# loicland/superpoint_graph

Measured on AMD Instinct MI355X. Metric: superpoints/sec (embed+ECC fwd+bwd), S3DIS-shaped SPG, higher is better.
Workload: dtype f32; 1 GPU; gru_10_0,f_13 fwd+bwd+Adam; 1 scene/GPU x 1000 sp x 128 pts x 14 f, 5000 edges x 13 f; hipgraph=False, step_call=spg_train_step (one library call: forward + backward), parallelism=single GPU, batchnorm=per-rank statistics, precision=f32

## Files before the change

### superpoint_graph_amd/csrc/spg_gemm.hip

```cpp
#pragma clang fp contract(off)
#include "../../include/spg_hip.h"
#include "spg_gemm.h"
#include <type_traits>
#include <float.h>
#include <limits.h>
#include <stdarg.h>

static thread_local char g_err[512] = "";
extern "C" const char* spg_last_error(void) { return g_err; }
void spg_set_error(const char* fmt, ...) {
  va_list ap;
  va_start(ap, fmt);
  vsnprintf(g_err, sizeof(g_err), fmt, ap);
  va_end(ap);
}

#include <mutex>
#include <vector>
#ifdef SPG_ATTRIBUTION
#define SPG_DBG(p) ((p).dbg)
#else
#define SPG_DBG(p) 0
#endif
namespace {
// ... 122 lines not shown
};
static_assert(sizeof(SpgMultiArgs) <= 4096, "kernel arguments of a grouped launch must fit 4 KiB");
static_assert(sizeof(SpgGemmParams) % 8 == 0 && sizeof(SpgWgradParams) % 8 == 0, "parameter structs are packed back to back");
constexpr int spg_gemm_variant(bool wred, int amode, bool full) {
  const int m = amode == -1 ? (full ? -1 : 4)
              : amode == SPG_PRO_IDENT ? (full ? 1 : 0)
              : ((!wred && amode == SPG_PRO_AFFINE) || (wred && amode == SPG_PRO_BNBWD)) ? (full ? 3 : 2) : -1;
  return m < 0 ? -1 : (wred ? 5 : 0) + m;
}
constexpr bool spg_gemm_variant_light(int v) { return v != 8; }
#define SPG_WGRAD_VARIANTS(X)                                                                                    \
  X(0, 128, 128, 2, 2, 3, 1, false, false, false)   X(1, 128, 128, 2, 2, 3, 1, true, false, false)               \
  X(2, 64, 64, 2, 2, 0, 1, false, true, true)       X(3, 64, 64, 2, 2, 0, 1, true, true, true)                   \
  X(4, 128, 64, 2, 2, 0, 1, false, false, false)    X(5, 128, 64, 2, 2, 0, 1, true, false, false)                \
  X(6, 128, 128, 2, 2, -1, -1, false, true, false)                                                               \
  X(7, 128, 32, 4, 1, 0, 0, false, false, true)     X(8, 128, 32, 4, 1, 0, 0, true, false, true)                 \
  X(9, 128, 32, 4, 1, -1, -1, false, true, false)                                                                \
  X(10, 128, 32, 4, 1, 0, 0, false, true, false)    X(11, 128, 32, 4, 1, 0, 0, true, true, true)                 \
  X(12, 128, 32, 4, 1, 0, 1, false, true, false)    X(13, 128, 32, 4, 1, 0, 1, true, true, false)                \
  X(14, 64, 64, 2, 2, 0, 1, false, false, true)     X(15, 64, 64, 2, 2, 0, 1, true, false, true)                 \
  X(16, 128, 128, 2, 2, 0, 1, false, true, false)   X(17, 128, 128, 2, 2, 0, 1, true, true, false)               \
  X(18, 128, 64, 2, 2, 3, 1, false, false, false)   X(19, 128, 64, 2, 2, 3, 1, true, false, false)
constexpr int spg_wgrad_variant(int it, int jt, int amode, int bmode, bool full, bool colsum) {
#define SPG_X(id, IT_, JT_, WI_, WJ_, AM_, BM_, FU_, CS_, LI_) \
  if (it == IT_ && jt == JT_ && amode == AM_ && bmode == BM_ && full == FU_ && colsum == CS_) return id;
  SPG_WGRAD_VARIANTS(SPG_X)
#undef SPG_X
  return -1;
}
constexpr bool spg_wgrad_variant_light(int v) {
#define SPG_X(id, IT_, JT_, WI_, WJ_, AM_, BM_, FU_, CS_, LI_) if (v == id) return LI_;
  SPG_WGRAD_VARIANTS(SPG_X)
#undef SPG_X
  return false;
}
static bool spg_group_accepts(hipStream_t stream);
static bool spg_group_add(int kind, int variant, const void* params, size_t bytes, dim3 grid, size_t lds, double flops, hipStream_t stream, int weight,
                          std::function<int()> direct = nullptr);

__device__ __forceinline__ int spg_opaque_zero() { int z = 0; asm volatile("" : "+v"(z)); return z; }
template <typename T> using spg_kernarg_ptr = __attribute__((address_space(4))) const T*;
template <int BYTES>
__device__ __forceinline__ void spg_touch_params(const spg_kernarg_ptr<unsigned> b) {
  unsigned acc = 0;
#pragma unroll
  for (int o = 0; o < BYTES; o += 64) acc |= b[o / 4];
  asm volatile("" :: "s"(acc));
}
#define SPG_EPI_PIECE_ROWS 16
#define SPG_EPI_WAVE_FLOATS(RW, CW) (SPG_EPI_PIECE_ROWS * ((CW) + 8))

template <int RW, int CW, int TI, int TJ>
__device__ __forceinline__ void spg_store_tile_vec_impl(const f32x16 (&acc)[TI][TJ], float* __restrict__ st,
                                                        float* __restrict__ ybase, unsigned ldy, int lane) {
  constexpr int LD = CW + 8, LPR = CW / 4, RPI = 64 / LPR;
  static_assert(SPG_EPI_PIECE_ROWS % RPI == 0, "a piece is a whole number of store instructions");
  const int r = lane & 31, h = lane >> 5;
  const int lr = lane / LPR, lc = 4 * (lane % LPR);
  const unsigned o0 = (unsigned)lr * ldy + (unsigned)lc;
#pragma unroll
  for (int i = 0; i < TI; ++i)
#pragma unroll
    for (int half = 0; half < 2; ++half) {
#pragma unroll
      for (int j = 0; j < TJ; ++j)
#pragma unroll
        for (int u = 0; u < 8; ++u) st[((u & 3) + 8 * (u >> 2) + 4 * h) * LD + 32 * j + r] = acc[i][j][8 * half + u];
#pragma unroll
      for (int it = 0; it < SPG_EPI_PIECE_ROWS / RPI; ++it) {
        const f32x4 v = *reinterpret_cast<const f32x4*>(st + (lr + RPI * it) * LD + lc);
        __builtin_nontemporal_store(v, reinterpret_cast<f32x4*>(ybase + o0 + (unsigned)(32 * i + 16 * half + RPI * it) * ldy));
      }
    }
}
template <int RW, int CW, int TI, int TJ>
__device__ __forceinline__ void spg_store_tile_vec(const f32x16 (&acc)[TI][TJ], float* __restrict__ st,
                                                   float* __restrict__ ybase, unsigned ldy, int lane) {
  static_assert(TI * 32 == RW && TJ * 32 == CW, "wave sub-tile");
  spg_store_tile_vec_impl<RW, CW, TI, TJ>(acc, st, ybase, ldy, lane);
}

#include "spg_fold.h"

template <int TJ>
struct SpgStatAcc {
  float n;
  float a[TJ], b[TJ];
  f32x4 s1, s2;
  float sg[TJ];
  bool has_sg;
};

template <int IT, int JT, int WI, int WJ, bool FULL, bool BIAS_DONE = false>
__device__ __forceinline__ void spg_epilogue_fwd(const SpgGemmParams& p, f32x16 (&acc)[IT / WI / 32][JT / WJ / 32],
                                                 float* __restrict__ red, int tile, long m0, int mvalid, int n0,
                                                 SpgStatAcc<JT / WJ / 32>& sacc, const bool accum, unsigned long long* edbg = nullptr) {
  constexpr int TI = IT / WI / 32, TJ = JT / WJ / 32;
  const int tid = threadIdx.x + spg_opaque_zero(), lane = tid & 63, wave = tid >> 6;
  const int r = lane & 31, h = lane >> 5;
  const int wi = wave / WJ, wj = wave % WJ;
  const int colw = wj * (JT / WJ), roww = wi * (IT / WI);
#ifdef SPG_ATTRIBUTION
  unsigned long long et__ = __builtin_readcyclecounter();
#define SPG_EP(k) if (edbg != nullptr) { const unsigned long long n__ = __builtin_readcyclecounter(); edbg[k] += n__ - et__; et__ = n__; }
#else
#define SPG_EP(k)
#endif
#pragma unroll
  for (int j = 0; j < TJ; ++j) {
    const int col = n0 + colw + 32 * j + r;
    const bool colok = FULL || col < p.N;
    if (!BIAS_DONE && p.bias != nullptr) {
      const float t = p.bias[colok ? col : 0];
      const float bv = colok ? t : 0.f;
#pragma unroll
      for (int i = 0; i < TI; ++i)
#pragma unroll
        for (int q = 0; q < 16; ++q) acc[i][j][q] += bv;
    }
    if (p.Y != nullptr && !(FULL && p.vec_store)) {
      float* yb = p.Y + m0 * p.ldy + n0;
      const unsigned ldy = (unsigned)p.ldy;
      const unsigned o0 = (unsigned)(roww + 4 * h) * ldy + (unsigned)(colw + 32 * j + r);
#pragma unroll
      for (int i = 0; i < TI; ++i)
#pragma unroll
        for (int q = 0; q < 16; ++q) {
          const int row = 32 * i + spg_acc_row(q, h);
          if (FULL || (colok && roww + row < mvalid)) yb[o0 + (unsigned)(32 * i + (q & 3) + 8 * (q >> 2)) * ldy] = acc[i][j][q];
        }
    }
  }
  if (FULL && p.vec_store && p.Y != nullptr) {
    spg_store_tile_vec<IT / WI, JT / WJ>(acc, red + wave * SPG_EPI_WAVE_FLOATS(IT / WI, JT / WJ),
                                         p.Y + (m0 + roww) * p.ldy + n0 + colw, (unsigned)p.ldy, lane);
  }
  SPG_EP(0);
  const int nvw = min(max(mvalid - roww, 0), IT / WI);
  const long part = (long)tile * WI + wi;
  if (p.stat != nullptr || p.stat_slots != nullptr) {
    const float inv = nvw > 0 ? 1.f / (float)nvw : 0.f;
#pragma unroll
    for (int j = 0; j < TJ; ++j) {
      const int col = n0 + colw + 32 * j + r;
      float s = 0.f;
#pragma unroll
      for (int i = 0; i < TI; ++i)
#pragma unroll
        for (int q = 0; q < 16; ++q)
          if (FULL || roww + 32 * i + spg_acc_row(q, h) < mvalid) s += acc[i][j][q];
      s += __shfl_xor(s, 32, 64);
      const float mean = s * inv;
      float m2 = 0.f;
      if constexpr (FULL) {
        const spg_f32x2 mean2 = {mean, mean};
#pragma unroll
        for (int i = 0; i < TI; ++i)
#pragma unroll
          for (int q = 0; q < 16; q += 2) {
            const spg_f32x2 d = spg_f32x2{acc[i][j][q], acc[i][j][q + 1]} - mean2;
            m2 = fmaf(d[0], d[0], m2);
            m2 = fmaf(d[1], d[1], m2);
          }
      } else {
#pragma unroll
        for (int i = 0; i < TI; ++i)
#pragma unroll
          for (int q = 0; q < 16; ++q)
            if (roww + 32 * i + spg_acc_row(q, h) < mvalid) {
              const float d = acc[i][j][q] - mean;
              m2 = fmaf(d, d, m2);
            }
      }
      m2 += __shfl_xor(m2, 32, 64);
      if (accum) {
        const float na = sacc.n, nb = (float)nvw, nn = na + nb;
        const float delta = mean - sacc.a[j], f = nn > 0.f ? nb / nn : 0.f;
        sacc.a[j] += delta * f;
        sacc.b[j] += m2 + delta * delta * (na * f);
      } else if (h == 0 && (FULL || col < p.N)) {
        if (p.stat_slots != nullptr) {
          if (nvw > 0) spg_slots_add_fwd(p.stat_slots, p.N, col, (float)nvw, mean, m2);
        } else {
          p.stat[(part * 2 + 0) * p.N + col] = mean;
          p.stat[(part * 2 + 1) * p.N + col] = m2;
        }
      }
    }
    if (accum) sacc.n += (float)nvw;
    else if (lane == 0 && wj == 0 && n0 == 0 && p.stat_slots == nullptr) p.stat_cnt[part] = (float)nvw;
  }
  SPG_EP(1);
  if (p.pool_out != nullptr) {
    float* xch = red + 4 * SPG_EPI_WAVE_FLOATS(IT / WI, JT / WJ);
    int* xci = reinterpret_cast<int*>(xch + WI * JT);
    float* xsg = xch + 2 * WI * JT;
#pragma unroll
    for (int j = 0; j < TJ; ++j) {
      const int cl = colw + 32 * j + r, col = n0 + cl;
      const bool colok = FULL || col < p.N;
      const float sg = sacc.has_sg ? (sacc.sg[j] < 0.f ? -1.f : 1.f) : ((p.pool_sign != nullptr && p.pool_sign[colok ? col : 0] < 0.f) ? -1.f : 1.f);
      float kb = -FLT_MAX;
      int ib = INT_MAX;
      const spg_f32x2 sg2 = {sg, sg};
#pragma unroll
      for (int i = 0; i < TI; ++i)
#pragma unroll
        for (int q2 = 0; q2 < 16; q2 += 2) {
          const spg_f32x2 key2 = spg_f32x2{acc[i][j][q2], acc[i][j][q2 + 1]} * sg2;
#pragma unroll
          for (int e = 0; e < 2; ++e) {
            const int q = q2 + e;
            const int row = roww + 32 * i + spg_acc_row(q, h);
            const float key = key2[e];
            const bool gt = (FULL || row < mvalid) && key > kb;
            kb = gt ? key : kb; ib = gt ? row : ib;
          }
        }
      const float ok = __shfl_xor(kb, 32, 64);
      const int oi = __shfl_xor(ib, 32, 64);
      if (ok > kb || (ok == kb && oi < ib)) { kb = ok; ib = oi; }
      if (h == 0) { xch[wi * JT + cl] = kb; xci[wi * JT + cl] = ib; if (wi == 0) xsg[cl] = sg; }
    }
    SPG_EP(2);
    __syncthreads();
    for (int cl = tid; cl < JT; cl += SPG_THREADS) {
      const int col = n0 + cl;
      if (!FULL && col >= p.N) continue;
      float kb = xch[cl];
      int ib = xci[cl];
#pragma unroll
      for (int w = 1; w < WI; ++w) {
        const float ok = xch[w * JT + cl];
        const int oi = xci[w * JT + cl];
        if (ok > kb || (ok == kb && oi < ib)) { kb = ok; ib = oi; }
      }
      const float sg = xsg[cl];
      p.pool_out[(long)tile * p.pool_ld + col] = kb * sg;
      if (p.pool_idx != nullptr) p.pool_idx[(long)tile * p.pool_ld + col] = ib;
    }
    if (n0 == 0 && p.pool_extra != nullptr)
      for (int e = tid; e < p.pool_nextra; e += SPG_THREADS)
        p.pool_out[(long)tile * p.pool_ld + p.N + e] = p.pool_extra[(long)tile * p.pool_nextra + e];
    SPG_EP(3);
  }
}

template <int IT, int JT, int WI, int WJ>
__device__ __forceinline__ void spg_bwd_stat_store(const SpgGemmParams& p, f32x4 s1, f32x4 s2, long part, int n0) {
  constexpr int CW = JT / WJ, LPR = CW / 4;
  const int tid = threadIdx.x + spg_opaque_zero(), lane = tid & 63, wave = tid >> 6;
  const int wj = wave % WJ;
  const int col = n0 + wj * CW + 4 * (lane % LPR);
#pragma unroll
  for (int off = LPR; off < 64; off <<= 1) {
#pragma unroll
    for (int e = 0; e < 4; ++e) { s1[e] += __shfl_xor(s1[e], off, 64); s2[e] += __shfl_xor(s2[e], off, 64); }
  }
  if (lane < LPR) {
    if (p.stat_slots != nullptr) {
#pragma unroll
      for (int e = 0; e < 4; ++e)
        if (col + e < p.n_mask) spg_slots_add(p.stat_slots, p.n_mask, col + e, (double)s1[e], (double)s2[e]);
    } else {
      *reinterpret_cast<f32x4*>(p.stat + (part * 2 + 0) * p.N + col) = s1;
      *reinterpret_cast<f32x4*>(p.stat + (part * 2 + 1) * p.N + col) = s2;
    }
  }
}

template <int IT, int JT, int WI, int WJ>
__device__ __forceinline__ void spg_epilogue_bwd_vec(const SpgGemmParams& p, f32x16 (&acc)[IT / WI / 32][JT / WJ / 32],
                                                     float* __restrict__ red, int tile, long m0, int n0,
                                                     SpgStatAcc<JT / WJ / 32>& sacc, const bool accum) {
  constexpr int TI = IT / WI / 32, TJ = JT / WJ / 32, RW = IT / WI, CW = JT / WJ;
  constexpr int LD = CW + 8, LPR = CW / 4, RPI = 64 / LPR, NIT = SPG_EPI_PIECE_ROWS / RPI;
  static_assert(SPG_EPI_PIECE_ROWS % RPI == 0, "a piece is a whole number of store instructions");
  const int tid = threadIdx.x + spg_opaque_zero(), lane = tid & 63, wave = tid >> 6;
  const int r = lane & 31, h = lane >> 5;
  const int wi = wave / WJ, wj = wave % WJ;
  const int colw = wj * CW, roww = wi * RW;
  float* st = red + wave * SPG_EPI_WAVE_FLOATS(RW, CW);
  const bool do_stats = (p.stat != nullptr || p.stat_slots != nullptr) && p.mmean != nullptr;
  const bool do_mask = p.mask_relu != 0 && p.Yp != nullptr;
  const bool use_y = p.Yp != nullptr && (do_stats || do_mask);
  const int lr = lane / LPR, lc = 4 * (lane % LPR);
  const int col = n0 + colw + lc;
  f32x4 sc = {1.f, 1.f, 1.f, 1.f}, sh = {0.f, 0.f, 0.f, 0.f}, mean = sh, rstd = sh;
  if (p.ms != nullptr) { sc = *reinterpret_cast<const f32x4*>(p.ms + col); sh = *reinterpret_cast<const f32x4*>(p.mt + col); }
  if (do_stats) { mean = *reinterpret_cast<const f32x4*>(p.mmean + col); rstd = *reinterpret_cast<const f32x4*>(p.mrstd + col); }
  const float* yp = p.Yp + (m0 + roww) * p.ldyp + n0 + colw;
  float* yo = p.Y + (m0 + roww) * p.ldy + n0 + colw;
  const unsigned op0 = (unsigned)lr * (unsigned)p.ldyp + (unsigned)lc, oo0 = (unsigned)lr * (unsigned)p.ldy + (unsigned)lc;
  f32x4 s1 = {0.f, 0.f, 0.f, 0.f}, s2 = s1;
#pragma unroll
  for (int i = 0; i < TI; ++i)
#pragma unroll
    for (int half = 0; half < 2; ++half) {
      const int rb = 32 * i + 16 * half;
      f32x4 yv[NIT];
      if (use_y) {
#pragma unroll
        for (int u = 0; u < NIT; ++u) yv[u] = *reinterpret_cast<const f32x4*>(yp + op0 + (unsigned)(rb + RPI * u) * (unsigned)p.ldyp);
      }
#pragma unroll
      for (int j = 0; j < TJ; ++j)
#pragma unroll
        for (int u = 0; u < 8; ++u) st[((u & 3) + 8 * (u >> 2) + 4 * h) * LD + 32 * j + r] = acc[i][j][8 * half + u];
#pragma unroll
      for (int u = 0; u < NIT; ++u) {
        f32x4 v = *reinterpret_cast<const f32x4*>(st + (lr + RPI * u) * LD + lc);
        const f32x4 y = use_y ? yv[u] : f32x4{0.f, 0.f, 0.f, 0.f};
        if (do_mask) {
          const f32x4 act = spg_fma4(y, sc, sh);
#pragma unroll
          for (int e = 0; e < 4; ++e)
            if (!(act[e] > 0.f)) v[e] = 0.f;
        }
        if (do_stats) {
          s1 += v;
          s2 = spg_fma4(v, (y - mean) * rstd, s2);
        }
// ... 3 lines not shown
    }
  if (accum) {
    sacc.s1 += s1; sacc.s2 += s2;
  } else if (p.stat != nullptr || p.stat_slots != nullptr) {
    spg_bwd_stat_store<IT, JT, WI, WJ>(p, s1, s2, (long)tile * WI + wi, n0);
  }
}

template <int IT, int JT, int WI, int WJ, bool FULL>
__device__ __forceinline__ void spg_epilogue_bwd(const SpgGemmParams& p, f32x16 (&acc)[IT / WI / 32][JT / WJ / 32],
                                                 float* __restrict__ red, int tile, long m0, int mvalid, int n0) {
  constexpr int TI = IT / WI / 32, TJ = JT / WJ / 32;
  const int tid = threadIdx.x + spg_opaque_zero(), lane = tid & 63, wave = tid >> 6;
  const int r = lane & 31, h = lane >> 5;
  const int wi = wave / WJ, wj = wave % WJ;
  const int colw = wj * (JT / WJ), roww = wi * (IT / WI);
  const bool do_stats = (p.stat != nullptr || p.stat_slots != nullptr) && p.mmean != nullptr;
  const bool do_mask = p.mask_relu != 0 && p.Yp != nullptr;
  const bool use_y = p.Yp != nullptr && (do_stats || do_mask);
#pragma unroll
  for (int j = 0; j < TJ; ++j) {
    const int col = n0 + colw + 32 * j + r;
    const bool colok = FULL || col < p.N;
    const bool inm = FULL || col < p.n_mask;
    const int cc = (colok && inm) ? col : 0;
    float sc = 1.f, sh = 0.f, mean = 0.f, rstd = 0.f;
    if (p.ms != nullptr) { sc = p.ms[cc]; sh = p.mt[cc]; }
    if (do_stats) { mean = p.mmean[cc]; rstd = p.mrstd[cc]; }
    const float* yp = p.Yp + m0 * p.ldyp + n0;
    float* yo = p.Y + m0 * p.ldy + n0;
    const unsigned ldyp = (unsigned)p.ldyp, ldyo = (unsigned)p.ldy;
    const unsigned cl = (unsigned)(colw + 32 * j + r);
    const unsigned op0 = (unsigned)(roww + 4 * h) * ldyp + (colok ? cl : 0u);
    const unsigned oo0 = (unsigned)(roww + 4 * h) * ldyo + cl;
    float s1 = 0.f, s2 = 0.f;
#pragma unroll
    for (int i = 0; i < TI; ++i) {
      float yv[16];
      if (use_y) {
#pragma unroll
        for (int q = 0; q < 16; ++q) {
          const int row = 32 * i + spg_acc_row(q, h);
          const bool ok = FULL || (colok && roww + row < mvalid);
          yv[q] = yp[ok ? op0 + (unsigned)(32 * i + (q & 3) + 8 * (q >> 2)) * ldyp : 0u];
        }
      }
#pragma unroll
      for (int q = 0; q < 16; ++q) {
        const int row = 32 * i + spg_acc_row(q, h);
        const bool ok = FULL || (colok && roww + row < mvalid);
        float v = acc[i][j][q];
        const float y = use_y ? yv[q] : 0.f;
        if (do_mask && inm && !(fmaf(y, sc, sh) > 0.f)) v = 0.f;
        if (FULL || ok) yo[oo0 + (unsigned)(32 * i + (q & 3) + 8 * (q >> 2)) * ldyo] = v;
        if (do_stats) {
          const float w = (ok && inm) ? v : 0.f;
          s1 += w;
          s2 = fmaf(w, (y - mean) * rstd, s2);
        }
      }
      __builtin_amdgcn_sched_barrier(0);
    }
    if (p.stat != nullptr || p.stat_slots != nullptr) {
      s1 += __shfl_xor(s1, 32, 64);
      s2 += __shfl_xor(s2, 32, 64);
      if (h == 0 && (FULL || col < p.N)) {
        const long part = (long)tile * WI + wi;
        if (p.stat_slots != nullptr) {
          if (col < p.n_mask) spg_slots_add(p.stat_slots, p.n_mask, col, (double)s1, (double)s2);
        } else {
          p.stat[(part * 2 + 0) * p.N + col] = s1;
          p.stat[(part * 2 + 1) * p.N + col] = s2;
        }
      }
    }
  }
}

template <int IT, int JT, int WI, int WJ, bool WRED, bool FULL, bool BIAS_DONE>
__device__ __forceinline__ void spg_tile_epilogue(const SpgGemmParams& p, f32x16 (&acc)[IT / WI / 32][JT / WJ / 32],
                                                  float* __restrict__ red, int tile, long m0, int mvalid, int n0,
                                                  SpgStatAcc<JT / WJ / 32>& sacc, const bool accum, unsigned long long* edbg = nullptr) {
  if constexpr (!WRED) {
    if (mvalid == IT && n0 + JT <= p.N) spg_epilogue_fwd<IT, JT, WI, WJ, true, BIAS_DONE>(p, acc, red, tile, m0, mvalid, n0, sacc, accum, edbg);
    else spg_epilogue_fwd<IT, JT, WI, WJ, false, BIAS_DONE>(p, acc, red, tile, m0, mvalid, n0, sacc, false);
  } else {
    const bool full = mvalid == IT && n0 + JT <= p.N && (n0 + JT <= p.n_mask || (p.stat == nullptr && p.stat_slots == nullptr && !p.mask_relu));
    if (FULL && full && p.vec_store) spg_epilogue_bwd_vec<IT, JT, WI, WJ>(p, acc, red, tile, m0, n0, sacc, accum);
    else if (full) spg_epilogue_bwd<IT, JT, WI, WJ, true>(p, acc, red, tile, m0, mvalid, n0);
    else spg_epilogue_bwd<IT, JT, WI, WJ, false>(p, acc, red, tile, m0, mvalid, n0);
  }
}

#ifdef SPG_ATTRIBUTION
__device__ unsigned long long spg_fwd_phase_t[4][14];
extern "C" int spg_fwd_phase_times(unsigned long long* out, int clear) {
  if (hipMemcpyFromSymbol(out, HIP_SYMBOL(spg_fwd_phase_t), sizeof(unsigned long long) * 56) != hipSuccess) return -1;
  if (clear) { unsigned long long z[56] = {0}; if (hipMemcpyToSymbol(HIP_SYMBOL(spg_fwd_phase_t), z, sizeof(z)) != hipSuccess) return -1; }
  return 0;
}
#define SPG_F0() unsigned long long ft__ = __builtin_readcyclecounter(), fp__[4] = {0, 0, 0, 0}, fn__ = 0, ep__[4] = {0, 0, 0, 0}, en__[4] = {0, 0, 0, 0}, et0__ = ft__
#define SPG_FP(k) { const unsigned long long n__ = __builtin_readcyclecounter(); fp__[k] += n__ - ft__; ft__ = n__; }
#define SPG_FTILE() ++fn__
#define SPG_FN(k) { const unsigned long long n__ = __builtin_readcyclecounter(); en__[k] += n__ - et0__; et0__ = n__; }
#define SPG_FN_FIRST(k) if (fn__ == 0) SPG_FN(k)
#define SPG_FEND() if (STREAM && !WRED && threadIdx.x == 0) { const int c__ = p.N > 128 ? 2 : (p.K > 64 ? 1 : (p.pool_out != nullptr ? 3 : 0)); \
    for (int k__ = 0; k__ < 4; ++k__) atomicAdd(&spg_fwd_phase_t[c__][k__], fp__[k__]); atomicAdd(&spg_fwd_phase_t[c__][4], 1ull); atomicAdd(&spg_fwd_phase_t[c__][5], fn__); for (int k__ = 0; k__ < 4; ++k__) { atomicAdd(&spg_fwd_phase_t[c__][6 + k__], ep__[k__]); atomicAdd(&spg_fwd_phase_t[c__][10 + k__], en__[k__]); } }
#else
#define SPG_F0()
#define SPG_FP(k)
#define SPG_FTILE()
#define SPG_FN(k)
#define SPG_FN_FIRST(k)
#define SPG_FEND()
#endif

template <int IT, int JT, int WI, int WJ, bool WRED, int AMODE, bool FULL = false, bool STREAM = false, int PREC = 0>
__device__ __forceinline__ void spg_rowgemm_body(const SpgGemmParams& p, const int bx, const int by) {
  constexpr int TI = IT / WI / 32, TJ = JT / WJ / 32;
  static_assert(WI * WJ == 4 && TI >= 1 && TJ >= 1, "4 waves per workgroup");
  extern __shared__ f32x4 smem[];
  f32x4* As = smem;
  f32x4* Bs = smem + (SPG_KC / 4) * (IT + 1);
  float* Bsr = reinterpret_cast<float*>(Bs);

  SPG_F0();
  const int tid = threadIdx.x, lane = tid & 63, wave = tid >> 6;
  const int r = lane & 31, h = lane >> 5;
  const int wi = wave / WJ, wj = wave % WJ;
  constexpr int A_F4 = (SPG_KC / 4) * (IT + 1);
  constexpr int B_F4 = (WRED && PREC == 0) ? SPG_KC * (JT + 4) / 4 : (SPG_KC / 4) * (JT + 1);
  f32x16 acc[TI][TJ];

  if (p.stat_slots != nullptr && bx == 0 && by == 0 && threadIdx.x == 0)
    spg_slots_count_add(p.stat_slots, WRED ? p.n_mask : p.N, p.stat_rows != 0 ? p.stat_rows : (long)p.M);
  auto fold_now = [&]() __attribute__((always_inline)) {
    if constexpr (!WRED) {
      if (p.fold.slots != nullptr) spg_bn_fold_fwd(p.fold, bx == 0 && by == 0);
    } else {
      if (p.fold_bwd.slots != nullptr) spg_bn_fold_bwd(p.fold_bwd, false);
    }
  };
  if constexpr (!(AMODE >= 0 && FULL)) fold_now();

  if constexpr (AMODE >= 0 && FULL) {
    static_assert(4 * SPG_EPI_WAVE_FLOATS(IT / WI, JT / WJ) + 2 * WI * JT + JT <= 4 * (A_F4 + B_F4), "epilogue staging + pooling exchange must fit one LDS buffer");
    int tile = bx, ct = by;
    if (p.remap) {
      const int lin = bx, j = lin >> 3;
      ct = j % p.ncol;
      tile = (j / p.ncol) * 8 + (lin & 7);
    }
    const int ntile = p.ntile, rstride = p.rstride;
    if (tile >= ntile) return;
    const int n0 = ct * JT;
    long m0 = (long)tile * p.rows_per_tile;
    int mvalid = (int)min((long)p.rows_per_tile, (long)p.M - m0);
    constexpr bool BIAS_IN_ACC = !WRED;
    SpgStatAcc<TJ> sacc;
    sacc.n = 0.f;
#pragma unroll
    for (int j = 0; j < TJ; ++j) { sacc.a[j] = 0.f; sacc.b[j] = 0.f; }
    sacc.s1 = f32x4{0.f, 0.f, 0.f, 0.f}; sacc.s2 = sacc.s1;
    float bias_v[TJ];
    sacc.has_sg = !WRED && p.pool_out != nullptr;
#pragma unroll
    for (int j = 0; j < TJ; ++j) {
      const int col = n0 + wj * (JT / WJ) + 32 * j + r;
      bias_v[j] = 0.f; sacc.sg[j] = 1.f;
      if (BIAS_IN_ACC && p.bias != nullptr) bias_v[j] = p.bias[col < p.N ? col : 0];
      if (sacc.has_sg && p.pool_sign != nullptr) sacc.sg[j] = p.pool_sign[col < p.N ? col : 0];
    }
    SpgRowsFast<AMODE, IT> pa0, pa1;
    SpgWeightFast<JT> pw0, pw1;
    SpgWeightRedFast<JT> pwr0, pwr1;
    SpgWeightBf16<JT, PREC ? PREC : 1> pb0, pb1;
    constexpr int NIA = SpgRowsFast<AMODE, IT>::NI;
    constexpr int NIW = PREC ? SpgWeightBf16<JT, PREC ? PREC : 1>::NI : (WRED ? SpgWeightRedFast<JT>::NI : SpgWeightFast<JT>::NI);
    auto w_load = [&](SpgWeightFast<JT>& pw, SpgWeightRedFast<JT>& pwr, SpgWeightBf16<JT, PREC ? PREC : 1>& pb, int k, int i) __attribute__((always_inline)) {
      if constexpr (PREC != 0) pb.load_part(p.Wb, p.ldwb, n0, k, i);
      else if constexpr (WRED) pwr.load_part(p.W, p.ldw, n0, k, i);
      else pw.load_part(p.W, p.ldw, n0, k, i);
    };
    auto w_store = [&](const SpgWeightFast<JT>& pw, const SpgWeightRedFast<JT>& pwr, const SpgWeightBf16<JT, PREC ? PREC : 1>& pb, f32x4* B, int i) __attribute__((always_inline)) {
      if constexpr (PREC != 0) pb.store_part(B, i);
      else if constexpr (WRED) pwr.store_part(reinterpret_cast<float*>(B), i);
      else pw.store_part(B, i);
    };
    auto a_store = [&](const SpgRowsFast<AMODE, IT>& pa, f32x4* A, int i) __attribute__((always_inline)) {
      if constexpr (PREC != 0) pa.template store_part_bf16<PREC ? PREC : 1>(A, i);
      else pa.store_part(A, i);
    };
    static_assert(NIA + NIW + 4 <= SPG_KC / 2, "staging pieces must fit the MFMA slots of a chunk");
    const int nchunk = p.K / SPG_KC;
    pa0.init(p.a, mvalid); pa1.init(p.a, mvalid);
    if constexpr (PREC != 0) { pb0.init(p.ldwb, n0, p.N, p.wb_part_bytes); pb1.init(p.ldwb, n0, p.N, p.wb_part_bytes); }
    else if (WRED) { pwr0.init(p.ldw, n0, p.N); pwr1.init(p.ldw, n0, p.N); } else { pw0.init(p.ldw, n0, p.N); pw1.init(p.ldw, n0, p.N); }
    {
#pragma unroll
      for (int i = 0; i < NIA; ++i) pa0.load_part(p.a, m0, 0, i);
#pragma unroll
      for (int i = 0; i < NIW; ++i) w_load(pw0, pwr0, pb0, 0, i);
      SPG_FN(0);
      fold_now();
      SPG_FN(1);
      pa0.prepare(p.a, tile, 0);
#pragma unroll
      for (int i = 0; i < NIA; ++i) a_store(pa0, As, i);
#pragma unroll
      for (int i = 0; i < NIW; ++i) w_store(pw0, pwr0, pb0, Bs, i);
      const int k1 = nchunk > 1 ? SPG_KC : 0;
      pa1.prepare(p.a, tile, k1);
#pragma unroll
      for (int i = 0; i < NIA; ++i) pa1.load_part(p.a, m0, k1, i);
#pragma unroll
      for (int i = 0; i < NIW; ++i) w_load(pw1, pwr1, pb1, k1, i);
    }
    __syncthreads();
#pragma unroll
    for (int j = 0; j < TJ; ++j) asm volatile("" : "+v"(sacc.sg[j]), "+v"(bias_v[j]));
    SPG_FN(2);
    const int tile0 = tile;
    const bool accum = STREAM && (p.stat != nullptr || p.stat_slots != nullptr) && p.stat_accum;
    constexpr bool DEFER2 = WRED;
    for (;;) {
      tile = __builtin_amdgcn_readfirstlane(tile);
      m0 = (long)tile * p.rows_per_tile;
      const int nxt = tile + rstride;
      const bool has_next = STREAM && nxt < ntile;
      const long m0n = has_next ? (long)nxt * p.rows_per_tile : m0;
      const int tilen = has_next ? nxt : tile;
#pragma unroll
      for (int j = 0; j < TJ; ++j) {
        float bv = n0 + wj * (JT / WJ) + 32 * j + r < p.N ? bias_v[j] : 0.f;
        asm volatile("" : "+v"(bv));
        typedef double spg_f64x8 __attribute__((ext_vector_type(8)));
        const double bd = __builtin_bit_cast(double, spg_f32x2{bv, bv});
        const spg_f64x8 b8 = {bd, bd, bd, bd, bd, bd, bd, bd};
#pragma unroll
        for (int i = 0; i < TI; ++i) acc[i][j] = __builtin_bit_cast(f32x16, b8);
      }
      auto body = [&](int c, int k2, long ml, int tl, bool noload, SpgRowsFast<AMODE, IT>& paF, SpgWeightFast<JT>& pwF, SpgWeightRedFast<JT>& pwrF,
                      SpgWeightBf16<JT, PREC ? PREC : 1>& pbF, SpgRowsFast<AMODE, IT>& paL, SpgWeightFast<JT>& pwL, SpgWeightRedFast<JT>& pwrL,
                      SpgWeightBf16<JT, PREC ? PREC : 1>& pbL) __attribute__((always_inline)) {
        const int buf = c & 1;
// ... 3 lines not shown
        f32x4* Bn = Bs + (buf ^ 1) * (A_F4 + B_F4);
        auto piece = [&](int slot) __attribute__((always_inline)) {
          if (slot == 0) {
            if (!(DEFER2 && noload)) {
              paL.prepare(p.a, tl, k2);
#pragma unroll
              for (int i = 0; i < (NIA + 1) / 2; ++i) paL.load_part(p.a, ml, k2, i);
            }
          } else if (slot == 1) {
            if (!(DEFER2 && noload)) {
#pragma unroll
              for (int i = (NIA + 1) / 2; i < NIA; ++i) paL.load_part(p.a, ml, k2, i);
            }
          } else if (slot == 2) {
            if (!(DEFER2 && noload)) {
#pragma unroll
              for (int i = 0; i < NIW; ++i) w_load(pwL, pwrL, pbL, k2, i);
            }
          } else if (slot < 3 + NIA) {
            a_store(paF, An, slot - 3);
          } else if (slot < 3 + NIA + NIW) {
            w_store(pwF, pwrF, pbF, Bn, slot - 3 - NIA);
          }
        };
        if constexpr (PREC != 0) {
          int sa[TI], sb[TJ];
#pragma unroll
          for (int i = 0; i < TI; ++i) sa[i] = wi * (IT / WI) + r + 32 * i;
#pragma unroll
          for (int j = 0; j < TJ; ++j) sb[j] = wj * (JT / WJ) + r + 32 * j;
          spg_mfma_chunk_bf16_il<TI, TJ, PREC>(Ac, Bc, IT + 1, JT + 1, sa, sb, h, acc, piece);
        }
        else if (WRED) spg_mfma_chunk_or_il<TI, TJ>(Ac, reinterpret_cast<const float*>(Bc), IT + 1, JT + 4, wi * (IT / WI) + r, wj * (JT / WJ) + r, h, acc, piece);
        else spg_mfma_chunk_il<TI, TJ>(Ac, Bc, IT + 1, JT + 1, wi * (IT / WI) + r, wj * (JT / WJ) + r, h, acc, piece);
        if (!(STREAM && (SPG_DBG(p) & 32))) __syncthreads();
      };
      const int reps = STREAM ? 1 + ((SPG_DBG(p) >> 8) & 15) : 1;
      SPG_FN_FIRST(3);
      SPG_FP(fn__ == 0 ? 0 : 2);
      for (int rep = 0; rep < reps; ++rep)
      for (int c = 0; c < nchunk; c += 2) {
        int ka = c + 2, kb = c + 3;
        long ma = m0, mb = m0;
        if (STREAM && (SPG_DBG(p) & 16)) ma = mb = (long)(tile & 15) * p.rows_per_tile;
        int ta = tile, tb = tile;
        if (ka >= nchunk) { if (has_next) { ka -= nchunk; ma = (STREAM && (SPG_DBG(p) & 16)) ? ma : m0n; ta = tilen; } else ka = nchunk - 1; }
        if (kb >= nchunk) { if (has_next) { kb -= nchunk; mb = (STREAM && (SPG_DBG(p) & 16)) ? mb : m0n; tb = tilen; } else kb = nchunk - 1; }
        body(c, ka * SPG_KC, ma, ta, false, pa1, pw1, pwr1, pb1, pa0, pw0, pwr0, pb0);
        if (c + 1 < nchunk) body(c + 1, kb * SPG_KC, mb, tb, has_next && c + 2 >= nchunk, pa0, pw0, pwr0, pb0, pa1, pw1, pwr1, pb1);
      }
      float* red = reinterpret_cast<float*>(smem + (A_F4 + B_F4));
      SPG_FP(1); SPG_FTILE();
      if (STREAM && SPG_DBG(p)) {
        if (SPG_DBG(p) & 8) {
          if (acc[0][0][0] + acc[TI - 1][TJ - 1][5] == 123.456f) p.Y[0] = 0.f;
        } else {
          SpgGemmParams q = p;
          if (SPG_DBG(p) & 1) q.Y = nullptr;
          if (SPG_DBG(p) & 2) q.stat = nullptr;
          if (SPG_DBG(p) & 4) q.pool_out = nullptr;
          spg_tile_epilogue<IT, JT, WI, WJ, WRED, true, BIAS_IN_ACC>(q, acc, red, tile, m0, mvalid, n0, sacc, false);
        }
      } else
#ifdef SPG_ATTRIBUTION
      spg_tile_epilogue<IT, JT, WI, WJ, WRED, true, BIAS_IN_ACC>(p, acc, red, tile, m0, mvalid, n0, sacc, accum, ep__);
#else
      spg_tile_epilogue<IT, JT, WI, WJ, WRED, true, BIAS_IN_ACC>(p, acc, red, tile, m0, mvalid, n0, sacc, accum);
#endif
      if (!has_next) break;
      tile = nxt; m0 = m0n;
      if (DEFER2) {
        pa1.prepare(p.a, tile, SPG_KC);
#pragma unroll
        for (int i = 0; i < NIA; ++i) pa1.load_part(p.a, m0, SPG_KC, i);
#pragma unroll
        for (int i = 0; i < NIW; ++i) w_load(pw1, pwr1, pb1, SPG_KC, i);
      }
      __syncthreads();
    }
    SPG_FP(2);
    if (accum) {
      float* xch = reinterpret_cast<float*>(smem);
      const long part = tile0;
      __syncthreads();
      if constexpr (!WRED) {
        if (wi != 0 && h == 0) {
#pragma unroll
          for (int j = 0; j < TJ; ++j) {
            const int cl = wj * (JT / WJ) + 32 * j + r;
            xch[(wi * JT + cl) * 2 + 0] = sacc.a[j];
            xch[(wi * JT + cl) * 2 + 1] = sacc.b[j];
          }
        }
        __syncthreads();
        if (wi == 0 && h == 0) {
          const float nb = sacc.n;
#pragma unroll
          for (int j = 0; j < TJ; ++j) {
            const int cl = wj * (JT / WJ) + 32 * j + r, col = n0 + cl;
            float na = sacc.n, mean = sacc.a[j], m2 = sacc.b[j];
#pragma unroll
            for (int w = 1; w < WI; ++w) {
              const float nn = na + nb, f = nn > 0.f ? nb / nn : 0.f;
              const float delta = xch[(w * JT + cl) * 2 + 0] - mean;
              mean += delta * f;
              m2 += xch[(w * JT + cl) * 2 + 1] + delta * delta * (na * f);
              na = nn;
            }
            if (col < p.N) {
              if (p.stat_slots != nullptr) {
                spg_slots_add_fwd(p.stat_slots, p.N, col, na, mean, m2);
              } else {
                p.stat[(part * 2 + 0) * p.N + col] = mean;
                p.stat[(part * 2 + 1) * p.N + col] = m2;
              }
            }
          }
          if (lane == 0 && wj == 0 && n0 == 0 && p.stat_slots == nullptr) p.stat_cnt[part] = sacc.n * (float)WI;
        }
      } else {
        constexpr int CW = JT / WJ, LPR = CW / 4;
        f32x4 s1 = sacc.s1, s2 = sacc.s2;
#pragma unroll
        for (int off = LPR; off < 64; off <<= 1) {
#pragma unroll
          for (int e = 0; e < 4; ++e) { s1[e] += __shfl_xor(s1[e], off, 64); s2[e] += __shfl_xor(s2[e], off, 64); }
        }
        const int cl = wj * CW + 4 * (lane % LPR);
        if (wi != 0 && lane < LPR) {
          *reinterpret_cast<f32x4*>(xch + (wi * JT + cl) * 2) = s1;
          *reinterpret_cast<f32x4*>(xch + (wi * JT + cl) * 2 + 4) = s2;
        }
        __syncthreads();
        if (wi == 0 && lane < LPR) {
#pragma unroll
          for (int w = 1; w < WI; ++w) {
            s1 += *reinterpret_cast<const f32x4*>(xch + (w * JT + cl) * 2);
            s2 += *reinterpret_cast<const f32x4*>(xch + (w * JT + cl) * 2 + 4);
          }
          if (p.stat_slots != nullptr) {
#pragma unroll
            for (int e = 0; e < 4; ++e)
              if (n0 + cl + e < p.n_mask) spg_slots_add(p.stat_slots, p.n_mask, n0 + cl + e, (double)s1[e], (double)s2[e]);
          } else {
            *reinterpret_cast<f32x4*>(p.stat + (part * 2 + 0) * p.N + n0 + cl) = s1;
            *reinterpret_cast<f32x4*>(p.stat + (part * 2 + 1) * p.N + n0 + cl) = s2;
          }
        }
      }
    }
    SPG_FP(3); SPG_FEND();
    return;
  }

  const int tile = bx;
  const long m0 = (long)tile * p.rows_per_tile;
  const int mvalid = (int)min((long)p.rows_per_tile, (long)p.M - m0);
  const int n0 = by * JT;
#pragma unroll
  for (int i = 0; i < TI; ++i)
#pragma unroll
    for (int j = 0; j < TJ; ++j)
#pragma unroll
      for (int q = 0; q < 16; ++q) acc[i][j][q] = 0.f;
  if constexpr (AMODE >= 0) {
    SpgRowsPipe<AMODE, IT> pa;
    SpgWeightPipe<JT> pw;
    SpgWeightRedPipe<JT> pwr;
    constexpr int NIA = SpgRowsPipe<AMODE, IT>::NI;
    constexpr int NIW = WRED ? SpgWeightRedPipe<JT>::NI : SpgWeightPipe<JT>::NI;
    static_assert(NIA + NIW + 4 <= SPG_KC / 2, "staging pieces must fit the MFMA slots of a chunk");
    const int nchunk = (p.K + SPG_KC - 1) / SPG_KC;
    pa.load(p.a, m0, mvalid, 0, p.K);
    if (WRED) pwr.load(p.W, p.ldw, n0, p.N, 0, p.K); else pw.load(p.W, p.ldw, n0, p.N, 0, p.K);
    pa.store(As);
    if (WRED) pwr.store(Bsr); else pw.store(Bs);
    {
      const int k1 = nchunk > 1 ? SPG_KC : 0;
      pa.load(p.a, m0, mvalid, k1, p.K);
      if (WRED) pwr.load(p.W, p.ldw, n0, p.N, k1, p.K); else pw.load(p.W, p.ldw, n0, p.N, k1, p.K);
    }
    __syncthreads();
    for (int c = 0; c < nchunk; ++c) {
      const int k2 = (c + 2 < nchunk ? c + 2 : nchunk - 1) * SPG_KC;
      const int buf = c & 1;
      const f32x4* Ac = As + buf * (A_F4 + B_F4);
      const f32x4* Bc = Bs + buf * (A_F4 + B_F4);
      f32x4* An = As + (buf ^ 1) * (A_F4 + B_F4);
      f32x4* Bn = Bs + (buf ^ 1) * (A_F4 + B_F4);
      auto piece = [&](int slot) __attribute__((always_inline)) {
        if (slot < NIA) {
          pa.store_part(An, slot);
        } else if (slot < NIA + NIW) {
          if (WRED) pwr.store_part(reinterpret_cast<float*>(Bn), slot - NIA); else pw.store_part(Bn, slot - NIA);
        } else if (slot == NIA + NIW) {
          pa.prepare(p.a, k2, p.K);
#pragma unroll
          for (int i = 0; i < (NIA + 1) / 2; ++i) pa.load_part(p.a, m0, mvalid, i);
        } else if (slot == NIA + NIW + 1) {
#pragma unroll
          for (int i = (NIA + 1) / 2; i < NIA; ++i) pa.load_part(p.a, m0, mvalid, i);
        } else if (slot == NIA + NIW + 2) {
#pragma unroll
// ... 62 lines not shown
      for (int e = 0; e < 8; ++e) v[e] = k0 + e < j.K ? j.W[n * j.ldw + k0 + e] : 0.f;
      out = (char*)j.fwd + (n * ldk + k0) * 2;
      part = (long)j.N * ldk * 2;
    } else {
      const long t = u - ufwd, k = t / (ldn / 8), n0 = 8 * (t % (ldn / 8));
#pragma unroll
      for (int e = 0; e < 8; ++e) v[e] = n0 + e < j.N ? j.W[(n0 + e) * j.ldw + k] : 0.f;
      out = (char*)j.bwd + (k * ldn + n0) * 2;
      part = (long)j.K * ldn * 2;
    }
    u32x2 h0, l0, h1, l1;
    spg_split_bf16(f32x4{v[0], v[1], v[2], v[3]}, h0, l0);
    spg_split_bf16(f32x4{v[4], v[5], v[6], v[7]}, h1, l1);
    *reinterpret_cast<uint4*>(out) = uint4{h0[0], h0[1], h1[0], h1[1]};
    *reinterpret_cast<uint4*>(out + part) = uint4{l0[0], l0[1], l1[0], l1[1]};
  }
}

int spg_launch_split_weights(const SpgSplitBatch& b, hipStream_t stream) {
  if (b.njobs == 0) return 0;
  hipLaunchKernelGGL(spg_split_weights_kernel, dim3(64, b.njobs), dim3(256), 0, stream, b);
  SPG_LAUNCH_CHECK();
  return 0;
}

int spg_gemm_precision() { return g_tune[SPG_TUNE_PRECISION]; }

int spg_gemm_ntiles(const SpgGemmParams& p) { return spg_cdiv(p.M, p.rows_per_tile); }

int spg_gemm_row_waves(int rows_per_tile, int N) {
  if (rows_per_tile <= 32) return 1;
  if (N <= 32) return 4;
  return 2;
}

template <int IT, int JT, int WI, int WJ, bool WRED, int AMODE>
static int launch_gemm_t(const SpgGemmParams& p, hipStream_t stream, int* stat_parts) {
  size_t lds = (size_t)(SPG_KC / 4) * (IT + 1) * sizeof(f32x4) +
               (WRED ? (size_t)SPG_KC * (JT + 4) * sizeof(float) : (size_t)(SPG_KC / 4) * (JT + 1) * sizeof(f32x4));
  if (AMODE >= 0) lds *= 2;
  size_t epi = (size_t)4 * WI * JT * sizeof(float);
  const size_t epi_vec = ((size_t)4 * SPG_EPI_WAVE_FLOATS(IT / WI, JT / WJ) + (size_t)2 * WI * JT) * sizeof(float);
  if (epi < epi_vec) epi = epi_vec;
  if (lds < epi) lds = epi;
  dim3 grid(spg_gemm_ntiles(p), spg_cdiv(p.N, JT));
  if (stat_parts != nullptr) *stat_parts = (int)grid.x * WI;
  const double flops = 2.0 * (double)p.M * (double)p.N * (double)p.K;
  const bool grouped = IT == 32 && spg_group_accepts(stream);
  ProfScope prof(stream, flops, 0, !grouped);
  prof.r.M = p.M; prof.r.N = p.N; prof.r.K = p.K;
  if constexpr (AMODE >= 0) {
    const bool mode_ok = AMODE == SPG_PRO_IDENT || AMODE == SPG_PRO_BNBWD ||
                         (AMODE == SPG_PRO_AFFINE && p.a.c0 != nullptr && p.a.n_affine >= p.K) ||
                         (AMODE == SPG_PRO_POOLBWD && p.a.P == IT && p.rows_per_tile == IT && p.M % IT == 0);
    const bool full = mode_ok && p.K % SPG_KC == 0 && (!WRED || (p.N & 3) == 0) &&
                      (long)IT * p.a.ld < (1L << 29) && (long)(WRED ? SPG_KC : JT) * p.ldw < (1L << 29);
    if (full) {
      SpgGemmParams q = p;
      q.vec_store = p.Y != nullptr && (p.ldy & 3) == 0 && (((uintptr_t)p.Y) & 15) == 0;
      if (WRED)
        q.vec_store = q.vec_store && (p.N & 3) == 0 && (p.Yp == nullptr || ((p.ldyp & 3) == 0 && (((uintptr_t)p.Yp) & 15) == 0)) &&
                      ((((uintptr_t)p.ms) | ((uintptr_t)p.mt) | ((uintptr_t)p.mmean) | ((uintptr_t)p.mrstd) | ((uintptr_t)p.stat)) & 15) == 0;
      prof.r.tag = SPG_PROF_TAG(1, IT, JT, WRED ? 1 : 0, AMODE, 1);
      q.ntile = (int)grid.x; q.rstride = 1 << 30; q.remap = 0; q.ncol = (int)grid.y;
      const int slots = 2 * spg_num_cus();
      const int ncol = (int)grid.y;
      const int prec = (IT == 128 && q.Wb != nullptr) ? g_tune[SPG_TUNE_PRECISION] : 0;
      if (!g_tune[SPG_TUNE_NO_PERSIST] && IT == 128 && !(WRED && JT == 128) && p.rows_per_tile == IT && p.M % IT == 0 && p.N % JT == 0 &&
          (p.K / SPG_KC) % 2 == 0 && (long)grid.x * ncol > slots && slots % (8 * ncol) == 0) {
        q.remap = 1; q.rstride = slots / ncol;
#ifdef SPG_ATTRIBUTION
        q.dbg = WRED ? 0 : g_tune[SPG_TUNE_DBG];
#else
        q.dbg = 0;
#endif
#ifndef SPG_ATTRIBUTION
        const int no_stat_accum = 0;
#else
        const int no_stat_accum = g_tune[SPG_TUNE_NO_STAT_ACCUM];
#endif
        q.stat_accum = !no_stat_accum && (p.stat != nullptr || p.stat_slots != nullptr) && (!WRED || (q.vec_store && p.N <= p.n_mask));
        if (q.stat_accum && stat_parts != nullptr) *stat_parts = (int)(q.rstride < q.ntile ? q.rstride : q.ntile);
        grid = dim3((unsigned)slots, 1);
        if constexpr (IT == 128 && !(WRED && JT == 128)) {
          if (prec == 3) hipLaunchKernelGGL((spg_rowgemm_kernel<IT, JT, WI, WJ, WRED, AMODE, true, true, 3>), grid, dim3(SPG_THREADS), lds, stream, q);
          else if (prec == 1) hipLaunchKernelGGL((spg_rowgemm_kernel<IT, JT, WI, WJ, WRED, AMODE, true, true, 1>), grid, dim3(SPG_THREADS), lds, stream, q);
          else hipLaunchKernelGGL((spg_rowgemm_kernel<IT, JT, WI, WJ, WRED, AMODE, true, true>), grid, dim3(SPG_THREADS), lds, stream, q);
          SPG_LAUNCH_CHECK();
          return 0;
        }
      }
      if constexpr (IT == 128 && WRED && JT == 128) {
        if (prec != 0) {
          if (prec == 3) hipLaunchKernelGGL((spg_rowgemm_kernel<IT, JT, WI, WJ, WRED, AMODE, true, false, 3>), grid, dim3(SPG_THREADS), lds, stream, q);
          else hipLaunchKernelGGL((spg_rowgemm_kernel<IT, JT, WI, WJ, WRED, AMODE, true, false, 1>), grid, dim3(SPG_THREADS), lds, stream, q);
          SPG_LAUNCH_CHECK();
          return 0;
        }
      }
      if constexpr (IT == 32 && spg_gemm_variant(WRED, AMODE, true) >= 0) {
        if (grouped && spg_group_add(SPG_JOB_GEMM, spg_gemm_variant(WRED, AMODE, true), &q, sizeof(q), grid, lds, flops, stream, 2 + 2 * spg_cdiv(p.K, SPG_KC),
                                     [q, grid, lds, stream]() -> int {
                                       hipLaunchKernelGGL((spg_rowgemm_kernel<IT, JT, WI, WJ, WRED, AMODE, true, false>), grid, dim3(SPG_THREADS), lds, stream, q);
                                       SPG_LAUNCH_CHECK();
                                       return 0;
                                     })) return 0;
      }
      hipLaunchKernelGGL((spg_rowgemm_kernel<IT, JT, WI, WJ, WRED, AMODE, true, false>), grid, dim3(SPG_THREADS), lds, stream, q);
      SPG_LAUNCH_CHECK();
      return 0;
    }
  }
  prof.r.tag = SPG_PROF_TAG(1, IT, JT, WRED ? 1 : 0, AMODE, 0);
  SpgGemmParams pv = p;
  pv.vec_store = !WRED && p.Y != nullptr && (p.ldy & 3) == 0 && (((uintptr_t)p.Y) & 15) == 0;
  if constexpr (IT == 32 && spg_gemm_variant(WRED, AMODE, false) >= 0) {
    if (grouped && spg_group_add(SPG_JOB_GEMM, spg_gemm_variant(WRED, AMODE, false), &pv, sizeof(pv), grid, lds, flops, stream, 2 + 2 * spg_cdiv(p.K, SPG_KC),
                                 [pv, grid, lds, stream]() -> int {
                                   hipLaunchKernelGGL((spg_rowgemm_kernel<IT, JT, WI, WJ, WRED, AMODE>), grid, dim3(SPG_THREADS), lds, stream, pv);
                                   SPG_LAUNCH_CHECK();
                                   return 0;
                                 })) return 0;
  }
  hipLaunchKernelGGL((spg_rowgemm_kernel<IT, JT, WI, WJ, WRED, AMODE>), grid, dim3(SPG_THREADS), lds, stream, pv);
  SPG_LAUNCH_CHECK();
  return 0;
}

template <bool WRED, int AMODE>
static int launch_gemm_shape(const SpgGemmParams& p, hipStream_t stream, int* sp) {
  if (p.rows_per_tile <= 32) return launch_gemm_t<32, 128, 1, 4, WRED, AMODE>(p, stream, sp);
  if (p.N <= 32) return launch_gemm_t<128, 32, 4, 1, WRED, AMODE>(p, stream, sp);
  if (p.N <= 64) return launch_gemm_t<128, 64, 2, 2, WRED, AMODE>(p, stream, sp);
  return launch_gemm_t<128, 128, 2, 2, WRED, AMODE>(p, stream, sp);
}

static int spg_launch_gemm_impl(const SpgGemmParams& p, hipStream_t stream, int* stat_parts);
static long group_njobs();
int spg_launch_gemm(const SpgGemmParams& p, hipStream_t stream, int* stat_parts) {
  if (p.stat_slots == nullptr || !spg_slot_sync_active()) return spg_launch_gemm_impl(p, stream, stat_parts);
  const long before = group_njobs();
  SPG_TRY(spg_launch_gemm_impl(p, stream, stat_parts));
  const int C = p.w_red ? p.n_mask : p.N;
  return spg_slot_sync_after(p.stat_slots, spg_fold_slot_words(C), stream, group_njobs() > before);
}
static int spg_launch_gemm_impl(const SpgGemmParams& p, hipStream_t stream, int* stat_parts) {
  SPG_CHECK_ARG(p.M > 0 && p.N > 0 && p.K > 0, "empty GEMM");
  SPG_CHECK_ARG(p.rows_per_tile >= 1 && p.rows_per_tile <= 128, "rows_per_tile must be in [1,128]");
  SPG_CHECK_ARG(p.epi == SPG_EPI_FWD || p.Y != nullptr, "backward epilogue needs an output");
  SPG_CHECK_ARG((p.epi == SPG_EPI_BWD) == (p.w_red != 0), "forward epilogue <-> [N,K] weights, backward epilogue <-> [K,N] weights");
  SPG_CHECK_ARG(p.epi != SPG_EPI_FWD || p.stat == nullptr || p.stat_cnt != nullptr, "forward statistics need stat_cnt");
  SPG_CHECK_ARG(p.stat_slots == nullptr || p.stat == nullptr, "statistics slots replace the partials");
  SPG_CHECK_ARG(p.fold.slots == nullptr || (p.epi == SPG_EPI_FWD && !p.w_red), "a statistics fold belongs to a forward launch");
  const bool walign = (p.ldw & 3) == 0 && (((uintptr_t)p.W) & 15) == 0 && p.ldw >= (((p.w_red ? p.N : p.K) + 3) & ~3);
  const bool vec = spg_operand_vec_ok(p.a) && walign && p.a.ld >= ((p.K + 3) & ~3);
  const int mode = vec ? p.a.mode : -1;
  if (!p.w_red) {
    if (p.a.mode == SPG_PRO_CLOUD && p.rows_per_tile > 32 && p.N > 32 && p.N <= 64)
      return launch_gemm_t<128, 64, 2, 2, false, -2>(p, stream, stat_parts);
    switch (mode) {
      case SPG_PRO_IDENT: return launch_gemm_shape<false, SPG_PRO_IDENT>(p, stream, stat_parts);
      case SPG_PRO_AFFINE: return launch_gemm_shape<false, SPG_PRO_AFFINE>(p, stream, stat_parts);
      default: return launch_gemm_shape<false, -1>(p, stream, stat_parts);
    }
  }
  switch (mode) {
// ... 1811 lines not shown
```

Baseline: 925,700 superpoints/s.

## Use 1x4 strip wave layout for pooled forward GEMM to drop cross-wave reductions

Adds a strip wave layout (WI=1, WJ=4) for the 128x128 persistent forward GEMM with max-pooling. Each wave then owns a full column strip of the tile, so the max-pool and batch-norm statistics no longer need an LDS exchange and __syncthreads between row waves. Each wave keeps two half-tile Welford accumulators and merges them in registers. In exchange each wave holds a 4x1 accumulator grid, which raises register pressure and changes the B-operand reuse pattern.

```diff
diff --git a/superpoint_graph_amd/csrc/spg_gemm.hip b/superpoint_graph_amd/csrc/spg_gemm.hip
--- a/superpoint_graph_amd/csrc/spg_gemm.hip
+++ b/superpoint_graph_amd/csrc/spg_gemm.hip
@@ -228,10 +228,13 @@
 
 #include "spg_fold.h"
 
+__host__ __device__ constexpr bool spg_strip_layout(int IT, int WI) { return WI == 1 && IT == 128; }
+
 template <int TJ>
 struct SpgStatAcc {
   float n;
   float a[TJ], b[TJ];
+  float a2[TJ], b2[TJ];
   f32x4 s1, s2;
   float sg[TJ];
   bool has_sg;
@@ -242,6 +245,8 @@
                                                  float* __restrict__ red, int tile, long m0, int mvalid, int n0,
                                                  SpgStatAcc<JT / WJ / 32>& sacc, const bool accum, unsigned long long* edbg = nullptr) {
   constexpr int TI = IT / WI / 32, TJ = JT / WJ / 32;
+  constexpr bool STRIP = spg_strip_layout(IT, WI);
+  static_assert(!STRIP || FULL, "the strip layout serves whole tiles only");
   const int tid = threadIdx.x + spg_opaque_zero(), lane = tid & 63, wave = tid >> 6;
   const int r = lane & 31, h = lane >> 5;
   const int wi = wave / WJ, wj = wave % WJ;
@@ -284,6 +289,57 @@
   SPG_EP(0);
   const int nvw = min(max(mvalid - roww, 0), IT / WI);
   const long part = (long)tile * WI + wi;
+  if constexpr (STRIP) {
+    if (p.stat != nullptr || p.stat_slots != nullptr) {
+      constexpr float nb = (float)(IT / 2), inv = 1.f / nb;
+#pragma unroll
+      for (int j = 0; j < TJ; ++j) {
+        const int col = n0 + colw + 32 * j + r;
+        float hm[2], hq[2];
+#pragma unroll
+        for (int hh = 0; hh < 2; ++hh) {
+          float s = 0.f;
+#pragma unroll
+          for (int i = 2 * hh; i < 2 * hh + 2; ++i)
+#pragma unroll
+            for (int q = 0; q < 16; ++q) s += acc[i][j][q];
+          s += __shfl_xor(s, 32, 64);
+          const float mean = s * inv;
+          float m2 = 0.f;
+          const spg_f32x2 mean2 = {mean, mean};
+#pragma unroll
+          for (int i = 2 * hh; i < 2 * hh + 2; ++i)
+#pragma unroll
+            for (int q = 0; q < 16; q += 2) {
+              const spg_f32x2 d = spg_f32x2{acc[i][j][q], acc[i][j][q + 1]} - mean2;
+              m2 = fmaf(d[0], d[0], m2);
+              m2 = fmaf(d[1], d[1], m2);
+            }
+          m2 += __shfl_xor(m2, 32, 64);
+          hm[hh] = mean; hq[hh] = m2;
+        }
+        if (accum) {
+          const float na = sacc.n, nn = na + nb, f = nn > 0.f ? nb / nn : 0.f;
+          const float d0 = hm[0] - sacc.a[j], d1 = hm[1] - sacc.a2[j];
+          sacc.a[j] += d0 * f;
+          sacc.b[j] += hq[0] + d0 * d0 * (na * f);
+          sacc.a2[j] += d1 * f;
+          sacc.b2[j] += hq[1] + d1 * d1 * (na * f);
+        } else if (h == 0) {
+          const float nn = nb + nb, f = nb / nn, delta = hm[1] - hm[0];
+          const float mean = hm[0] + delta * f, m2 = hq[0] + (hq[1] + delta * delta * (nb * f));
+          if (p.stat_slots != nullptr) {
+            spg_slots_add_fwd(p.stat_slots, p.N, col, nn, mean, m2);
+          } else {
+            p.stat[(part * 2 + 0) * p.N + col] = mean;
+            p.stat[(part * 2 + 1) * p.N + col] = m2;
+          }
+        }
+      }
+      if (accum) sacc.n += nb;
+      else if (lane == 0 && wj == 0 && n0 == 0 && p.stat_slots == nullptr) p.stat_cnt[part] = (float)IT;
+    }
+  } else
   if (p.stat != nullptr || p.stat_slots != nullptr) {
     const float inv = nvw > 0 ? 1.f / (float)nvw : 0.f;
 #pragma unroll
@@ -366,24 +422,33 @@
       const float ok = __shfl_xor(kb, 32, 64);
       const int oi = __shfl_xor(ib, 32, 64);
       if (ok > kb || (ok == kb && oi < ib)) { kb = ok; ib = oi; }
-      if (h == 0) { xch[wi * JT + cl] = kb; xci[wi * JT + cl] = ib; if (wi == 0) xsg[cl] = sg; }
+      if constexpr (STRIP) {
+        if (h == 0) {
+          p.pool_out[(long)tile * p.pool_ld + col] = kb * sg;
+          if (p.pool_idx != nullptr) p.pool_idx[(long)tile * p.pool_ld + col] = ib;
+        }
+      } else {
+        if (h == 0) { xch[wi * JT + cl] = kb; xci[wi * JT + cl] = ib; if (wi == 0) xsg[cl] = sg; }
+      }
     }
     SPG_EP(2);
-    __syncthreads();
-    for (int cl = tid; cl < JT; cl += SPG_THREADS) {
-      const int col = n0 + cl;
-      if (!FULL && col >= p.N) continue;
-      float kb = xch[cl];
-      int ib = xci[cl];
-#pragma unroll
-      for (int w = 1; w < WI; ++w) {
-        const float ok = xch[w * JT + cl];
-        const int oi = xci[w * JT + cl];
-        if (ok > kb || (ok == kb && oi < ib)) { kb = ok; ib = oi; }
-      }
-      const float sg = xsg[cl];
-      p.pool_out[(long)tile * p.pool_ld + col] = kb * sg;
-      if (p.pool_idx != nullptr) p.pool_idx[(long)tile * p.pool_ld + col] = ib;
+    if constexpr (!STRIP) {
+      __syncthreads();
+      for (int cl = tid; cl < JT; cl += SPG_THREADS) {
+        const int col = n0 + cl;
+        if (!FULL && col >= p.N) continue;
+        float kb = xch[cl];
+        int ib = xci[cl];
+#pragma unroll
+        for (int w = 1; w < WI; ++w) {
+          const float ok = xch[w * JT + cl];
+          const int oi = xci[w * JT + cl];
+          if (ok > kb || (ok == kb && oi < ib)) { kb = ok; ib = oi; }
+        }
+        const float sg = xsg[cl];
+        p.pool_out[(long)tile * p.pool_ld + col] = kb * sg;
+        if (p.pool_idx != nullptr) p.pool_idx[(long)tile * p.pool_ld + col] = ib;
+      }
     }
     if (n0 == 0 && p.pool_extra != nullptr)
       for (int e = tid; e < p.pool_nextra; e += SPG_THREADS)
@@ -553,8 +618,8 @@
                                                   float* __restrict__ red, int tile, long m0, int mvalid, int n0,
                                                   SpgStatAcc<JT / WJ / 32>& sacc, const bool accum, unsigned long long* edbg = nullptr) {
   if constexpr (!WRED) {
-    if (mvalid == IT && n0 + JT <= p.N) spg_epilogue_fwd<IT, JT, WI, WJ, true, BIAS_DONE>(p, acc, red, tile, m0, mvalid, n0, sacc, accum, edbg);
-    else spg_epilogue_fwd<IT, JT, WI, WJ, false, BIAS_DONE>(p, acc, red, tile, m0, mvalid, n0, sacc, false);
+    if (spg_strip_layout(IT, WI) || (mvalid == IT && n0 + JT <= p.N)) spg_epilogue_fwd<IT, JT, WI, WJ, true, BIAS_DONE>(p, acc, red, tile, m0, mvalid, n0, sacc, accum, edbg);
+    else if constexpr (!spg_strip_layout(IT, WI)) spg_epilogue_fwd<IT, JT, WI, WJ, false, BIAS_DONE>(p, acc, red, tile, m0, mvalid, n0, sacc, false);
   } else {
     const bool full = mvalid == IT && n0 + JT <= p.N && (n0 + JT <= p.n_mask || (p.stat == nullptr && p.stat_slots == nullptr && !p.mask_relu));
     if (FULL && full && p.vec_store) spg_epilogue_bwd_vec<IT, JT, WI, WJ>(p, acc, red, tile, m0, n0, sacc, accum);
@@ -631,7 +696,7 @@
     SpgStatAcc<TJ> sacc;
     sacc.n = 0.f;
 #pragma unroll
-    for (int j = 0; j < TJ; ++j) { sacc.a[j] = 0.f; sacc.b[j] = 0.f; }
+    for (int j = 0; j < TJ; ++j) { sacc.a[j] = 0.f; sacc.b[j] = 0.f; sacc.a2[j] = 0.f; sacc.b2[j] = 0.f; }
     sacc.s1 = f32x4{0.f, 0.f, 0.f, 0.f}; sacc.s2 = sacc.s1;
     float bias_v[TJ];
     sacc.has_sg = !WRED && p.pool_out != nullptr;
@@ -801,8 +866,31 @@
     if (accum) {
       float* xch = reinterpret_cast<float*>(smem);
       const long part = tile0;
-      __syncthreads();
-      if constexpr (!WRED) {
+      if constexpr (!WRED && spg_strip_layout(IT, WI)) {
+        if (h == 0) {
+          const float nb = sacc.n;
+#pragma unroll
+          for (int j = 0; j < TJ; ++j) {
+            const int col = n0 + wj * (JT / WJ) + 32 * j + r;
+            float na = sacc.n, mean = sacc.a[j], m2 = sacc.b[j];
+            const float nn = na + nb, f = nn > 0.f ? nb / nn : 0.f;
+            const float delta = sacc.a2[j] - mean;
+            mean += delta * f;
+            m2 += sacc.b2[j] + delta * delta * (na * f);
+            na = nn;
+            if (col < p.N) {
+              if (p.stat_slots != nullptr) {
+                spg_slots_add_fwd(p.stat_slots, p.N, col, na, mean, m2);
+              } else {
+                p.stat[(part * 2 + 0) * p.N + col] = mean;
+                p.stat[(part * 2 + 1) * p.N + col] = m2;
+              }
+            }
+          }
+          if (lane == 0 && wj == 0 && n0 == 0 && p.stat_slots == nullptr) p.stat_cnt[part] = sacc.n * 2.f;
+        }
+      } else if constexpr (!WRED) {
+        __syncthreads();
         if (wi != 0 && h == 0) {
 #pragma unroll
           for (int j = 0; j < TJ; ++j) {
@@ -838,6 +926,7 @@
           if (lane == 0 && wj == 0 && n0 == 0 && p.stat_slots == nullptr) p.stat_cnt[part] = sacc.n * (float)WI;
         }
       } else {
+        __syncthreads();
         constexpr int CW = JT / WJ, LPR = CW / 4;
         f32x4 s1 = sacc.s1, s2 = sacc.s2;
 #pragma unroll
@@ -1066,6 +1155,15 @@
         q.stat_accum = !no_stat_accum && (p.stat != nullptr || p.stat_slots != nullptr) && (!WRED || (q.vec_store && p.N <= p.n_mask));
         if (q.stat_accum && stat_parts != nullptr) *stat_parts = (int)(q.rstride < q.ntile ? q.rstride : q.ntile);
         grid = dim3((unsigned)slots, 1);
+        if constexpr (IT == 128 && JT == 128 && WI == 2 && !WRED) {
+          if (p.pool_out != nullptr && (q.stat_accum || (p.stat == nullptr && p.stat_slots == nullptr))) {
+            if (prec == 3) hipLaunchKernelGGL((spg_rowgemm_kernel<IT, JT, 1, 4, WRED, AMODE, true, true, 3>), grid, dim3(SPG_THREADS), lds, stream, q);
+            else if (prec == 1) hipLaunchKernelGGL((spg_rowgemm_kernel<IT, JT, 1, 4, WRED, AMODE, true, true, 1>), grid, dim3(SPG_THREADS), lds, stream, q);
+            else hipLaunchKernelGGL((spg_rowgemm_kernel<IT, JT, 1, 4, WRED, AMODE, true, true>), grid, dim3(SPG_THREADS), lds, stream, q);
+            SPG_LAUNCH_CHECK();
+            return 0;
+          }
+        }
         if constexpr (IT == 128 && !(WRED && JT == 128)) {
           if (prec == 3) hipLaunchKernelGGL((spg_rowgemm_kernel<IT, JT, WI, WJ, WRED, AMODE, true, true, 3>), grid, dim3(SPG_THREADS), lds, stream, q);
           else if (prec == 1) hipLaunchKernelGGL((spg_rowgemm_kernel<IT, JT, WI, WJ, WRED, AMODE, true, true, 1>), grid, dim3(SPG_THREADS), lds, stream, q);
```

Result: no change. 926,100 superpoints/s (median of 3 runs) (+0.0%).
